# ps-auxw/CLI-P

Hardware: AMD Instinct MI355X
Metric: images/sec ViT-B/32 encode (higher is better)
Workload: dtype bf16

## Files before the change

cli-p_amd/csrc/encode.hip:

```cpp
#include "vit_kernels.hpp"

namespace clipmi {
namespace {

struct Ws {
    unsigned short* patches;
    float* x;
    unsigned short* h;
    unsigned short* big;
    unsigned short* pooled;
    int* rowidx;
    unsigned char* a8;
    float* a_scale;
    unsigned char* a_bs;
    unsigned char* x8;
    unsigned char* x8_bs;
    void* x3;
    float* ln_part;
    float* ln_leaf;
    void* x3c;
    float* partc;
    float* leafc;
    float* xc;
};
// ... 41 lines not shown
    if (t->abi_version != CLIPMI_ABI_VERSION)
        return set_err(CLIPMI_EINVAL, "%s: tower ABI %d != %d", who, t->abi_version, CLIPMI_ABI_VERSION);
    if (t->kind != kind) return set_err(CLIPMI_EINVAL, "%s: tower kind %d", who, t->kind);
    if (t->width % 128 != 0 || t->heads * 64 != t->width || t->mlp != 4 * t->width || t->embed % 128 != 0 ||
        t->width > 1024 || t->layers < 1)
        return set_err(CLIPMI_EUNSUPPORTED,
                       "%s: width=%d heads=%d mlp=%d embed=%d (need width %% 128 == 0 <= 1024, head dim 64, embed %% 128 == 0)",
                       who, t->width, t->heads, t->mlp, t->embed);
    if (t->weight_format != 0 && t->weight_format != 1)
        return set_err(CLIPMI_EINVAL, "%s: weight_format %d", who, t->weight_format);
    if (t->weight_format == 1 && t->width % 256 != 0)
        return set_err(CLIPMI_EUNSUPPORTED, "%s: fp8 weights need width %% 256 == 0 (width %d)", who, t->width);
    if (t->ln_fold != 0 && (t->ln_fold != 1 || t->width % 256 != 0))
        return set_err(CLIPMI_EINVAL, "%s: ln_fold %d needs width %% 256 == 0 (width %d)", who, t->ln_fold, t->width);
#ifndef CLIPMI_DEV
    if (t->ln_fold != 0 && t->weight_format != 0)
        return set_err(CLIPMI_EUNSUPPORTED, "%s: folded LayerNorms on FP8 weights exist in the development library only", who);
#endif
    if (t->tokens > 80 && kind == 1)
        return set_err(CLIPMI_EUNSUPPORTED, "%s: %d tokens (causal attention covers <= 80)", who, t->tokens);
    return 0;
}

template <typename T>
const T* at(const void* blob, uint64_t off) {
    return reinterpret_cast<const T*>(static_cast<const char*>(blob) + off);
}

bool encode_tail() {
    static const int mode = (int)dev_knob("CLIPMI_ENCODE_TAIL", 1);
    return mode != 0;
}

int launch_gather_rows(const void* src, void* dst, int B, int L, size_t row_bytes, hipStream_t st) {
    if (row_bytes % 16 != 0) return set_err(CLIPMI_EINVAL, "gather_rows: %zu bytes per row", row_bytes);
    const int row16 = (int)(row_bytes / 16);
    hipLaunchKernelGGL(gather_rows_kernel, dim3((unsigned)(((long long)B * row16 + 255) / 256)), dim3(256), 0, st,
                       static_cast<const uint4*>(src), static_cast<uint4*>(dst), B, L, row16);
    CLIPMI_CHECK_LAUNCH("gather_rows_kernel");
    return 0;
}

struct LayerW {
    const unsigned short *qkv_w, *out_w, *fc_w, *proj_w;
    const float *qkv_b, *out_b, *fc_b, *proj_b, *qkv_colsum, *fc_colsum, *qkv_s, *out_s, *fc_s, *proj_s, *ln1_w, *ln1_b, *ln2_w, *ln2_b;
    LayerW(const clipmi_tower* t, const void* blob, int l) {
        const uint64_t lb = t->off_layers + (uint64_t)l * t->layer_stride;
        auto f = [&](uint64_t lo) { return at<float>(blob, lb + lo); };
        auto h = [&](uint64_t lo) { return at<unsigned short>(blob, lb + lo); };
        qkv_w = h(t->lo_qkv_w); out_w = h(t->lo_out_w); fc_w = h(t->lo_fc_w); proj_w = h(t->lo_proj_w);
        qkv_b = f(t->ln_fold ? t->lo_qkv_cb : t->lo_qkv_b); fc_b = f(t->ln_fold ? t->lo_fc_cb : t->lo_fc_b);
        out_b = f(t->lo_out_b); proj_b = f(t->lo_proj_b); qkv_colsum = f(t->lo_qkv_colsum); fc_colsum = f(t->lo_fc_colsum);
        qkv_s = f(t->lo_qkv_s); out_s = f(t->lo_out_s); fc_s = f(t->lo_fc_s); proj_s = f(t->lo_proj_s);
        ln1_w = f(t->lo_ln1_w); ln1_b = f(t->lo_ln1_b); ln2_w = f(t->lo_ln2_w); ln2_b = f(t->lo_ln2_b);
    }
};

GemmArgs linear(const void* A, size_t lda_bytes, const unsigned short* W, const float* bias, int M, int N, int K, void* out) {
    GemmArgs g{};
    g.A = static_cast<const unsigned short*>(A); g.lda_bytes = (unsigned)lda_bytes; g.W = W; g.bias = bias;
    g.M = M; g.N = N; g.K = K; g.out = out;
    return g;
}

struct Resid { const float* x; const void* x3; long long row_step; };

// ... 1 lines not shown
    const clipmi_tower* t; const void* blob; const Ws& w; int B, causal; hipStream_t st; GemmProbe* probe; bool tail; int W, L, M, last;
};

int tail_plain(const Blocks& c, const LayerW& lw, Resid& r) {
    const Ws& w = c.w; const int B = c.B, W = c.W;
    if (int rc = launch_gather_rows(w.x, w.xc, B, c.L, (size_t)W * 4, c.st)) return rc;
    if (int rc = launch_gemm_algo(linear(w.h, (size_t)c.L * W * 2, lw.out_w, lw.out_b, B, W, W, w.xc), EPI_BIAS_RESID_F32, 0, c.st, nullptr)) return rc;
    LnArgs ln2{w.xc, lw.ln2_w, lw.ln2_b, w.h, nullptr, 1, B, W, 1};
    if (int rc = launch_layernorm(ln2, c.st)) return rc;
    if (int rc = launch_gemm_algo(linear(w.h, 0, lw.fc_w, lw.fc_b, B, 4 * W, W, w.big), EPI_BIAS_QGELU_BF16, 0, c.st, nullptr)) return rc;
    r = Resid{w.xc, nullptr, 1};
    return launch_gemm_algo(linear(w.big, 0, lw.proj_w, lw.proj_b, B, W, 4 * W, w.xc), EPI_BIAS_RESID_F32, 0, c.st, nullptr);
}

int blocks_plain(const Blocks& c, Resid& r) {
    const Ws& w = c.w; const int W = c.W, M = c.M;
    for (int l = 0; l <= c.last; ++l) {
        const LayerW lw(c.t, c.blob, l);
        LnArgs ln{w.x, lw.ln1_w, lw.ln1_b, w.h, nullptr, 1, M, W, 1};
        if (int rc = launch_layernorm(ln, c.st)) return rc;
        if (int rc = launch_gemm_algo(linear(w.h, 0, lw.qkv_w, lw.qkv_b, M, 3 * W, W, w.big), EPI_BIAS_BF16, 0, c.st, c.probe)) return rc;
        if (int rc = launch_attention(w.big, w.h, c.B, c.L, c.t->heads, c.causal, ATTN_DEFAULT, c.st)) return rc;
        if (c.tail && l == c.last) return tail_plain(c, lw, r);
        if (int rc = launch_gemm_algo(linear(w.h, 0, lw.out_w, lw.out_b, M, W, W, w.x), EPI_BIAS_RESID_F32, 0, c.st, c.probe)) return rc;
        ln.w = lw.ln2_w; ln.b = lw.ln2_b;
        if (int rc = launch_layernorm(ln, c.st)) return rc;
        if (int rc = launch_gemm_algo(linear(w.h, 0, lw.fc_w, lw.fc_b, M, 4 * W, W, w.big), EPI_BIAS_QGELU_BF16, 0, c.st, c.probe)) return rc;
        if (int rc = launch_gemm_algo(linear(w.big, 0, lw.proj_w, lw.proj_b, M, W, 4 * W, w.x), EPI_BIAS_RESID_F32, 0, c.st, c.probe)) return rc;
    }
    return 0;
}

int tail_ln(const Blocks& c, const LayerW& lw, Resid& r) {
    const Ws& w = c.w; const int B = c.B, W = c.W;
    float* const leaf = w.leafc && gemm_resid_writes_leaves(B, W, W) && gemm_resid_writes_leaves(B, W, 4 * W) ? w.leafc : nullptr;
    if (int rc = launch_attention(w.big, w.h, B, c.L, c.t->heads, c.causal, ATTN_DEFAULT, c.st)) return rc;
    if (int rc = launch_gather_rows(w.x3, w.x3c, B, c.L, resid_row_bytes(W), c.st)) return rc;
    GemmArgs out = linear(w.h, (size_t)c.L * W * 2, lw.out_w, lw.out_b, B, W, W, nullptr);
    out.x3 = w.x3c; out.ln_part = w.partc; out.ln_leaf = leaf; out.tmp_f32 = w.x;
    if (int rc = launch_gemm_algo(out, EPI_BIAS_RESID_LN_F32, 0, c.st, nullptr)) return rc;
    GemmArgs fc = linear(w.x3c, resid_row_bytes(W), lw.fc_w, lw.fc_b, B, 4 * W, W, w.big);
    fc.colsum = lw.fc_colsum; fc.ln_part_in = w.partc; fc.ln_leaf_in = leaf;
    if (int rc = launch_gemm_algo(fc, EPI_LN_BIAS_QGELU_BF16, 0, c.st, nullptr)) return rc;
    GemmArgs proj = linear(w.big, 0, lw.proj_w, lw.proj_b, B, W, 4 * W, nullptr);
    proj.x3 = w.x3c; proj.ln_part = w.partc; proj.ln_leaf = leaf; proj.tmp_f32 = w.x;
    r = Resid{nullptr, w.x3c, 1};
    return launch_gemm_algo(proj, EPI_BIAS_RESID_LN_F32, 0, c.st, nullptr);
}

int blocks_ln(const Blocks& c, Resid& r) {
    const Ws& w = c.w; const int W = c.W, M = c.M;
    float* const leaf = w.ln_leaf && gemm_resid_writes_leaves(M, W, W) && gemm_resid_writes_leaves(M, W, 4 * W) ? w.ln_leaf : nullptr;
    const float* leaf_in = nullptr;
    for (int l = 0; l <= c.last; ++l) {
        const LayerW lw(c.t, c.blob, l);
        GemmArgs qkv = linear(w.x3, resid_row_bytes(W), lw.qkv_w, lw.qkv_b, M, 3 * W, W, w.big);
        qkv.colsum = lw.qkv_colsum; qkv.ln_part_in = w.ln_part; qkv.ln_leaf_in = leaf_in;
        if (int rc = launch_gemm_algo(qkv, EPI_LN_BIAS_BF16, 0, c.st, c.probe)) return rc;
        if (c.tail && l == c.last) return tail_ln(c, lw, r);
        hipEvent_t* aev = nullptr;
        if (c.probe && c.probe->mode == 2 && c.probe->n < GemmProbe::MAX) aev = &c.probe->ev[2 * c.probe->begin(GemmProbe::EPI_ATTENTION, 2, c.st, 0)];
        if (int rc = launch_attention(w.big, w.h, c.B, c.L, c.t->heads, c.causal, ATTN_DEFAULT, c.st, nullptr, nullptr, nullptr, aev)) return rc;
        GemmArgs out = linear(w.h, 0, lw.out_w, lw.out_b, M, W, W, nullptr);
        out.x3 = w.x3; out.ln_part = w.ln_part; out.ln_leaf = leaf; out.tmp_f32 = w.x;
        if (int rc = launch_gemm_algo(out, EPI_BIAS_RESID_LN_F32, 0, c.st, c.probe)) return rc;
        leaf_in = leaf;
        GemmArgs fc = linear(w.x3, resid_row_bytes(W), lw.fc_w, lw.fc_b, M, 4 * W, W, w.big);
        fc.colsum = lw.fc_colsum; fc.ln_part_in = w.ln_part; fc.ln_leaf_in = leaf_in;
        if (int rc = launch_gemm_algo(fc, EPI_LN_BIAS_QGELU_BF16, 0, c.st, c.probe)) return rc;
        GemmArgs proj = linear(w.big, 0, lw.proj_w, lw.proj_b, M, W, 4 * W, nullptr);
        proj.x3 = w.x3; proj.ln_part = w.ln_part; proj.ln_leaf = leaf; proj.tmp_f32 = w.x;
        if (int rc = launch_gemm_algo(proj, EPI_BIAS_RESID_LN_F32, 0, c.st, c.probe)) return rc;
    }
    return 0;
}

bool fp8_fuse_off() { static const bool off = dev_knob("CLIPMI_FP8_FUSE", 1) == 0; return off; }
int attention_fp8(const Blocks& c, const Ws& w) {
    bool fused = false;
    if (int rc = launch_attention(w.big, w.h, c.B, c.L, c.t->heads, c.causal, ATTN_DEFAULT, c.st, fp8_fuse_off() ? nullptr : w.a8, w.a_bs, &fused)) return rc;
// ... 46 lines not shown
        GemmArgs out = linear(w.a8, 0, lw.out_w, lw.out_b, M, W, W, w.x);
        out.a_bscale = w.a_bs; out.w_scale = lw.out_s; out.x8 = w.x8; out.x8_bs = w.x8_bs; out.ln_part = w.ln_part;
        if (int rc = launch_gemm_fp8(out, EPI_BIAS_RESID_LN8, c.st)) return rc;
        GemmArgs fc = linear(w.x8, 0, lw.fc_w, lw.fc_b, M, 4 * W, W, w.big);
        fc.a_bscale = w.x8_bs; fc.w_scale = lw.fc_s; fc.colsum = lw.fc_colsum; fc.ln_part_in = w.ln_part;
        const unsigned char* h8;
        if (int rc = fc_fp8(c, w, fc, EPI_LN_BIAS_QGELU_BF16, !fp8_fuse_off(), &h8)) return rc;
        GemmArgs proj = linear(h8, 0, lw.proj_w, lw.proj_b, M, W, 4 * W, w.x);
        proj.a_bscale = w.a_bs; proj.w_scale = lw.proj_s; proj.x8 = w.x8; proj.x8_bs = w.x8_bs; proj.ln_part = w.ln_part;
        if (int rc = launch_gemm_fp8(proj, EPI_BIAS_RESID_LN8, c.st)) return rc;
    }
    return 0;
}
#endif

int run_layers(const clipmi_tower* t, const void* blob, const Ws& w, int B, int causal, hipStream_t st, GemmProbe* probe, Resid* r) {
    const bool fp8 = t->weight_format == 1;
    const bool tail = !causal && !fp8 && (t->ln_fold ? w.x3c != nullptr : w.xc != nullptr) && encode_tail();
    const Blocks c{t, blob, w, B, causal, st, probe, tail, t->width, t->tokens, B * t->tokens, t->layers - 1};
    *r = Resid{w.x, w.x3, t->tokens};
#ifdef CLIPMI_DEV
    if (t->ln_fold && fp8) return blocks_ln_fp8(c);
#endif
    if (t->ln_fold) return blocks_ln(c, *r);
    return fp8 ? blocks_fp8(c) : blocks_plain(c, *r);
}

int run_head(const clipmi_tower* t, const void* blob, const Ws& w, const Resid& r, int B, const int* rowidx, float* out, int normalize, hipStream_t st) {
    const bool split = t->ln_fold && t->weight_format == 0;
    LnArgs ln{split ? nullptr : r.x, at<float>(blob, t->off_ln_post_w), at<float>(blob, t->off_ln_post_b), w.pooled, rowidx,
              r.row_step, B, t->width, 1};
    ln.x3 = r.x3;
    if (int rc = launch_layernorm(ln, st)) return rc;
    if (int rc = launch_gemm_algo(linear(w.pooled, 0, at<unsigned short>(blob, t->off_out_proj), nullptr, B, t->embed, t->width, out), EPI_F32, 0, st)) return rc;
    return normalize ? clipmi_l2_normalize_rows(out, B, t->embed, st) : 0;
}

}
}

using namespace clipmi;

extern "C" size_t clipmi_encode_image_workspace_bytes(const clipmi_tower* t, int B) {
    if (check_tower(t, 0, "encode_image")) return 0;
    if (B < 1) { set_err(CLIPMI_EINVAL, "encode_image: B=%d", B); return 0; }
    return carve(t, B, nullptr, ~(size_t)0, nullptr);
}

static int embed_image(const clipmi_tower* t, const void* blob_dev, const void* pixels_dev, int pix_dtype, int B, const Ws& w,
                       int algo, bool with_ln_pre, hipStream_t st) {
    const int W = t->width, L = t->tokens;
    const int grid = t->res / t->patch, np = grid * grid;
    PatchArgs pa{pixels_dev, w.patches, pix_dtype, B, t->res, t->patch, grid, np, t->patch_k};
    if (int rc = launch_patchify(pa, st)) return rc;
    GemmArgs g{};
    g.A = w.patches; g.W = at<unsigned short>(blob_dev, t->off_patch_w); g.bias = nullptr; g.out = w.x;
    g.M = B * np; g.N = W; g.K = t->patch_k; g.pos = at<float>(blob_dev, t->off_pos); g.np = np; g.L = L;
    if (int rc = launch_gemm_algo(g, EPI_PATCH_F32, algo, st)) return rc;
    hipLaunchKernelGGL(cls_rows_kernel, dim3((unsigned)(((long long)B * W + 255) / 256)), dim3(256), 0, st, w.x,
                       at<float>(blob_dev, t->off_cls), at<float>(blob_dev, t->off_pos), B, L, W);
    CLIPMI_CHECK_LAUNCH("cls_rows_kernel");
    if (!with_ln_pre) return 0;
    LnArgs ln{w.x, at<float>(blob_dev, t->off_ln_pre_w), at<float>(blob_dev, t->off_ln_pre_b), w.x, nullptr, 1, B * L, W, 0};
    const bool fold8 = t->ln_fold && t->weight_format == 1;
    if (t->ln_fold && !fold8) { ln.out_x3 = w.x3; ln.out_part = w.ln_part; }
    return launch_layernorm(ln, st);
}
// ... 208 lines not shown
```

cli-p_amd/csrc/gemm.hip:

```cpp
#include "gemm256p.hpp"
#include "gemm_skinny.hpp"
#include "gemm256f8.hpp"
#include <hip/hip_ext.h>
#include <cstdlib>
#include <type_traits>

namespace clipmi {

static_assert(plan_chip::NUM_CU == NUM_CU && plan_chip::LDS_BYTES == LDS_BYTES && plan_chip::G256_LDS == G256_LDS &&
              plan_chip::G256P_MAX_N == G256P_MAX_N, "gemm_plan.hpp restates these for host-only builds");

static const GemmKnobs& knobs() {
    static const GemmKnobs kn{(int)dev_knob("CLIPMI_GEMM_PERSIST", 1), (int)dev_knob("CLIPMI_GEMM_SPLIT", 40),
                              (int)dev_knob("CLIPMI_GEMM_SKINNY", 1), (int)dev_knob("CLIPMI_GEMM_GRID", NUM_CU)};
    return kn;
}

template <unsigned MASK, int E = 0, typename F>
static int with_epi(int epi, F&& f) {
    if constexpr (E <= EPI_BIAS_RESID_LN8) {
        if constexpr (epi_in(MASK, E))
            if (epi == E) return f(std::integral_constant<int, E>{});
        return with_epi<MASK, E + 1>(epi, f);
    }
    return set_err(CLIPMI_EINVAL, "gemm: epilogue %d is not built for this kernel", epi);
}

template <typename Kernel>
static void launch_probed(Kernel kernel, dim3 grid, dim3 block, int lds, hipStream_t st, GemmProbe* probe, int epi, int kernel_kind,
                          int K, const GemmArgs& g) {
    const int i = probe ? probe->begin(epi, kernel_kind, st, K) : 0;
    if (probe) hipExtLaunchKernelGGL(kernel, grid, block, lds, st, probe->ev[2 * i], probe->ev[2 * i + 1], 0, g);
    else hipLaunchKernelGGL(kernel, grid, block, lds, st, g);
}

static bool lds_opted(int* slots) {
    int dev = 0;
    (void)hipGetDevice(&dev);
    if (dev < 0 || dev >= 64) return false;
    if (slots[dev]) return true;
    slots[dev] = 1;
    return false;
}

template <auto KERNEL>
static int launch_g256(const GemmArgs& g, int grid, hipStream_t st, int lds_max, int lds, const char* opt_err, const char* name,
                       GemmProbe* probe = nullptr, int epi = 0, int kernel_kind = GK_256) {
// ... 4 lines not shown
    launch_probed(KERNEL, dim3(grid), dim3(512), lds, st, probe, epi, kernel_kind, g.K, g);
    CLIPMI_CHECK_LAUNCH(name);
    return 0;
}
static int grid256(const GemmArgs& g) { return (g.N / 256) * ((g.M + 255) / 256); }

template <int EPI>
static int launch_skinny(const GemmArgs& g, hipStream_t st) {
    const int nstrips = g.N / 16, mtiles = (g.M + 15) / 16;
    const int waves = nstrips * mtiles <= 4 * NUM_CU ? 1 : 4;
    const dim3 grid((nstrips + waves - 1) / waves, mtiles);
    if (g.K > 512) hipLaunchKernelGGL((gemm_skinny_kernel<EPI, 32>), grid, dim3(waves * 64), 0, st, g);
    else hipLaunchKernelGGL((gemm_skinny_kernel<EPI, 16>), grid, dim3(waves * 64), 0, st, g);
    CLIPMI_CHECK_LAUNCH("gemm_skinny_kernel");
    return 0;
}

static int launch_part(const GemmArgs& g, const GemmPart& part, hipStream_t st, GemmProbe* probe) {
    switch (part.kernel) {
        case GK_SKINNY:
            return with_epi<EPI_MASK_SKINNY>(part.epi, [&](auto e) { return launch_skinny<decltype(e)::value>(g, st); });
        case GK_128:
            return with_epi<EPI_MASK_128>(part.epi, [&](auto e) {
                constexpr int EPI = decltype(e)::value;
                launch_probed(gemm_bf16_nt_kernel<EPI>, dim3((g.N / GEMM_BN) * ((g.M + GEMM_BM - 1) / GEMM_BM)), dim3(256), GEMM_LDS_BYTES, st, probe, EPI, GK_128, g.K, g);
                CLIPMI_CHECK_LAUNCH("gemm_bf16_nt_kernel");
                return 0;
            });
        case GK_256:
            return with_epi<EPI_MASK_256>(part.epi, [&](auto e) {
                constexpr int EPI = decltype(e)::value;
                return launch_g256<gemm256_bf16_nt_kernel<EPI>>(g, grid256(g), st, G256_LDS, G256_LDS, "hipFuncSetAttribute(gemm256, %d B LDS)",
                                                                "gemm256_bf16_nt_kernel", probe, EPI);
            });
        default:
            return with_epi<EPI_MASK_256P>(part.epi, [&](auto e) {
                constexpr int EPI = decltype(e)::value;
                return launch_g256<gemm256p_bf16_nt_kernel<EPI, false>>(g, part.grid, st, LDS_BYTES, part.lds, "hipFuncSetAttribute(gemm256p, %d B LDS)",
                                                                        "gemm256p_bf16_nt_kernel", probe, EPI, GK_256P);
            });
    }
}

static GemmArgs gemm_rows(const GemmArgs& g, int epi, int row0, int rows) {
    GemmArgs b = g;
    b.M = rows;
    b.A = g.A + (size_t)row0 * gemm_lda(g);
    const size_t oe = (size_t)row0 * g.N;
    if (epi == EPI_BIAS_RESID_LN_F32) {
        b.x3 = static_cast<char*>(g.x3) + (size_t)row0 * resid_row_bytes(g.N); b.tmp_f32 = g.tmp_f32 + oe;
        b.ln_part = g.ln_part + (size_t)row0 * (g.N / 256) * 2;
    } else {
        b.out = static_cast<char*>(g.out) + oe * (epi_is_bf16_out(epi) ? 2 : 4);
    }
    if (b.ln_part_in) b.ln_part_in = g.ln_part_in + (size_t)row0 * (g.K / 256) * 2;
    return b;
}

bool gemm_resid_writes_leaves(int M, int N, int K) {
    const GemmPlan p = gemm_plan(M, N, K, EPI_BIAS_RESID_LN_F32, 0, true, false, 0, knobs());
    return !p.err && p.nparts == 1 && p.part[0].leaves;
}

int launch_gemm_algo(const GemmArgs& g, int epi, int algo, hipStream_t st, GemmProbe* probe) {
    if (epi_is_ln(epi) && ((!g.ln_part_in && !g.ln_leaf_in) || !g.colsum || !g.bias))
        return set_err(CLIPMI_EINVAL, "gemm: LN-folded epilogue %d needs ln_part_in, colsum, bias and K %% 256 == 0, K <= 1024", epi);
// ... 32 lines not shown
                                                                                      "gemm256p_bf16_nt_kernel");
            });
        case GK_F8_BSA:
            return with_epi<EPI_MASK_FP8_BSA>(epi, [&](auto e) {
                return launch_g256<gemm256f8_nt_kernel<decltype(e)::value, true, true>>(
                    g, grid256(g), st, G256_LDS + 256 * (plan_chip::FP8_BSA_MAX_K / 32), G256_LDS + 256 * (g.K / 32),
                    "hipFuncSetAttribute(gemm256f8 block-scaled)", "gemm256f8_nt_kernel(block-scaled A)");
            });
    }
    return with_epi<EPI_MASK_FP8>(epi, [&](auto e) {
        constexpr int EPI = decltype(e)::value;
        const char *opt_err = "hipFuncSetAttribute(gemm256f8, %d B LDS)", *name = "gemm256f8_nt_kernel";
        return mx ? launch_g256<gemm256f8_nt_kernel<EPI, true>>(g, grid256(g), st, G256_LDS, G256_LDS, opt_err, name)
                  : launch_g256<gemm256f8_nt_kernel<EPI, false>>(g, grid256(g), st, G256_LDS, G256_LDS, opt_err, name);
    });
}

bool gemm_fp8_emits_mx(int M, int N, int K) {
    const GemmPlan p = gemm_fp8_plan(M, N, K, EPI_BIAS_QGELU_BF16, 1, false, false, 0, knobs());
    return !p.err && p.part[0].kernel == GK_256P;
}

}

using namespace clipmi;

static GemmArgs hook_args(const void* a, const void* w, const float* bias, void* out, int M, int N, int K) {
    GemmArgs g{};
    g.A = static_cast<const unsigned short*>(a); g.W = static_cast<const unsigned short*>(w); g.bias = bias; g.out = out;
    g.M = M; g.N = N; g.K = K;
    return g;
}

extern "C" int clipmi_dbg_gemm_bf16(const void* a_dev, const void* w_dev, const float* bias_dev, void* out_dev, int M,
                                    int N, int K, int epi, void* stream) {
    const int algo = (epi >> 8) & 7;
    epi &= 0xff;
    if (epi < 0 || epi > 3) return set_err(CLIPMI_EINVAL, "dbg_gemm: epi %d", epi);
    GemmArgs g = hook_args(a_dev, w_dev, bias_dev, out_dev, M, N, K);
    static const int dbg_env = (int)dev_knob("CLIPMI_GEMM_DBG", 0);
    g.dbg = dbg_env;
    if (g.dbg & 12) { g.pos = bias_dev; g.bias = nullptr; }
    return launch_gemm_algo(g, epi, algo, as_stream(stream));
}

extern "C" int clipmi_dbg_gemm_ln(const void* x3_dev, const void* wg_dev, const float* cb_dev, const float* colsum_dev,
                                  const float* part_dev, void* out_dev, int M, int N, int K, int epi, void* stream) {
    const int algo = (epi >> 8) & 3;
    epi &= 0xff;
    if (!epi_is_ln(epi)) return set_err(CLIPMI_EINVAL, "dbg_gemm_ln: epi %d", epi);
    GemmArgs g = hook_args(x3_dev, wg_dev, cb_dev, out_dev, M, N, K);
    g.lda_bytes = (unsigned)resid_row_bytes(K); g.colsum = colsum_dev; g.ln_part_in = part_dev;
    return launch_gemm_algo(g, epi, algo, as_stream(stream));
}

extern "C" int clipmi_dbg_gemm_resid_ln_leaf(const void* a_dev, const void* w_dev, const float* bias_dev, void* x3_dev, float* leaf_dev,
                                             int M, int N, int K, void* stream) {
    if (!leaf_dev || !gemm_resid_writes_leaves(M, N, K))
        return set_err(CLIPMI_EINVAL, "dbg_gemm_resid_ln_leaf: M <= %d, N %% 256 == 0, N <= 1024, K %% 32 == 0", SKINNY_MAX_M);
    GemmArgs g = hook_args(a_dev, w_dev, bias_dev, nullptr, M, N, K);
    g.x3 = x3_dev; g.ln_leaf = leaf_dev;
    g.ln_part = leaf_dev; g.tmp_f32 = leaf_dev;
    return launch_gemm_algo(g, EPI_BIAS_RESID_LN_F32, 0, as_stream(stream));
}

extern "C" int clipmi_dbg_gemm_ln_leaf(const void* x3_dev, const void* wg_dev, const float* cb_dev, const float* colsum_dev,
                                       const float* leaf_dev, void* out_dev, int M, int N, int K, int epi, void* stream) {
    if (!epi_is_ln(epi)) return set_err(CLIPMI_EINVAL, "dbg_gemm_ln_leaf: epi %d", epi);
    GemmArgs g = hook_args(x3_dev, wg_dev, cb_dev, out_dev, M, N, K);
    g.lda_bytes = (unsigned)resid_row_bytes(K); g.colsum = colsum_dev; g.ln_leaf_in = leaf_dev;
    return launch_gemm_algo(g, epi, 0, as_stream(stream));
}

extern "C" int clipmi_dbg_gemm_resid_ln(const void* a_dev, const void* w_dev, const float* bias_dev, void* x3_dev,
                                        float* part_dev, float* tmp_dev, int M, int N, int K, int algo, void* stream) {
    GemmArgs g = hook_args(a_dev, w_dev, bias_dev, nullptr, M, N, K);
    g.x3 = x3_dev; g.ln_part = part_dev; g.tmp_f32 = tmp_dev;
    static const int dbg_env = (int)dev_knob("CLIPMI_GEMM_DBG", 0);
    g.dbg = dbg_env;
    return launch_gemm_algo(g, EPI_BIAS_RESID_LN_F32, algo & 7, as_stream(stream));
}

extern "C" int clipmi_dbg_gemm_fp8_bsa(const void* a8_dev, const void* w8_dev, const void* a_bscale_dev, const float* w_scale_dev,
                                       const float* bias_dev, void* out_dev, int M, int N, int K, int epi, void* stream) {
    GemmArgs g = hook_args(a8_dev, w8_dev, bias_dev, out_dev, M, N, K);
    g.a_bscale = static_cast<const unsigned char*>(a_bscale_dev); g.w_scale = w_scale_dev;
    return launch_gemm_fp8(g, epi, as_stream(stream), 1);
}

extern "C" int clipmi_dbg_gemm_fp8(const void* a8_dev, const void* w8_dev, const float* a_scale_dev, const float* w_scale_dev,
                                   const float* bias_dev, void* out_dev, int M, int N, int K, int epi, void* stream) {
    const int mx = (epi >> 8) & 1 ? 0 : ((epi >> 9) & 1 ? 2 : 1);
    epi &= 0xff;
    if (epi < 0 || epi > 3) return set_err(CLIPMI_EINVAL, "dbg_gemm_fp8: epi %d", epi);
    GemmArgs g = hook_args(a8_dev, w8_dev, bias_dev, out_dev, M, N, K);
    g.a_scale = a_scale_dev; g.w_scale = w_scale_dev;
    return launch_gemm_fp8(g, epi, as_stream(stream), mx);
}

extern "C" int clipmi_dbg_gemm_fp8_mxout(const void* a8_dev, const void* w8_dev, const float* a_scale_dev, const float* w_scale_dev,
                                         const float* bias_dev, void* out_dev, void* out_bscale_dev, int M, int N, int K, int epi,
                                         void* stream) {
    if (epi < 0 || epi > 3) return set_err(CLIPMI_EINVAL, "dbg_gemm_fp8_mxout: epi %d", epi);
    GemmArgs g = hook_args(a8_dev, w8_dev, bias_dev, out_dev, M, N, K);
    g.a_scale = a_scale_dev; g.w_scale = w_scale_dev; g.out_bscale = static_cast<unsigned char*>(out_bscale_dev);
    return launch_gemm_fp8(g, epi, as_stream(stream), 1);
}

static int plan_out(const GemmPlan& p, bool query, int32_t* out, int n_out) {
    if (!out || n_out < 1) return set_err(CLIPMI_EINVAL, "dbg_gemm_plan: no output array");
// ... 19 lines not shown
```

cli-p_amd/csrc/gemm_plan.hpp:

```cpp
#pragma once
#include <stdarg.h>
#include <stdio.h>
#include "../../include/clipmi.h"

namespace clipmi {

enum Epilogue {
    EPI_BIAS_BF16 = 0,
    EPI_BIAS_QGELU_BF16 = 1,
    EPI_BIAS_RESID_F32 = 2,
    EPI_F32 = 3,
    EPI_PATCH_F32 = 4,
    EPI_LN_BIAS_BF16 = 5,
    EPI_LN_BIAS_QGELU_BF16 = 6,
    EPI_BIAS_RESID_LN_F32 = 7,
    EPI_BIAS_RESID_LN8 = 8
};
constexpr bool epi_is_ln(int e) { return e == EPI_LN_BIAS_BF16 || e == EPI_LN_BIAS_QGELU_BF16; }
constexpr bool epi_is_qgelu(int e) { return e == EPI_BIAS_QGELU_BF16 || e == EPI_LN_BIAS_QGELU_BF16; }
constexpr bool epi_is_bf16_out(int e) { return e == EPI_BIAS_BF16 || e == EPI_BIAS_QGELU_BF16 || epi_is_ln(e); }

constexpr unsigned EPI_MASK_128 = 0x7f, EPI_MASK_256 = 0x7f;
constexpr unsigned EPI_MASK_256P = 0xe7, EPI_MASK_SKINNY = 0xff;
constexpr unsigned EPI_MASK_FP8 = 0x0f;
constexpr unsigned EPI_MASK_FP8_256P = 0x03;
#ifdef CLIPMI_DEV
constexpr unsigned EPI_MASK_FP8_BSA = 0x16c;
#else
constexpr unsigned EPI_MASK_FP8_BSA = 0x00c;
#endif
constexpr bool epi_in(unsigned mask, int e) { return e >= 0 && e < 32 && ((mask >> e) & 1u) != 0; }

namespace plan_chip {
constexpr int NUM_CU = 256, LDS_BYTES = 160 * 1024, G256_LDS = 128 * 1024, G256P_MAX_N = 8192, FP8_BSA_MAX_K = 4096;
}
constexpr int SKINNY_MAX_M = 128;

constexpr int g256p_lds(int epi, bool fp8, int N, int K, int dbg) {
    const int nseg = K >> 8;
    return plan_chip::G256_LDS + N * 4 * (fp8 ? 2 : 1) +
           (fp8 ? 1024 : epi_is_ln(epi) ? 1024 + 256 * nseg * 8 + (nseg < 4 ? 8 : 0) : 0) + ((dbg & 12) ? 8192 + 2048 : 0);
}

struct GemmKnobs {
    int persist = 1;
    int split = 40;
    int skinny = 1;
    int grid = plan_chip::NUM_CU;
};

enum GemmKernel { GK_128 = 0, GK_256 = 1, GK_256P = 2, GK_SKINNY = 3, GK_F8 = 4, GK_F8_BSA = 5 };

struct GemmPart {
    int rows, kernel, epi;
    bool scratch;
    bool leaves;
    int grid, lds;
};
struct GemmPlan {
    int err = 0;
    int nparts = 0;
    GemmPart part[3];
    char msg[224];
    GemmPlan& refuse(int code, const char* fmt, ...) __attribute__((format(printf, 3, 4))) {
        va_list ap; va_start(ap, fmt); vsnprintf(msg, sizeof(msg), fmt, ap); va_end(ap);
        err = code; return *this;
    }
    GemmPlan& add(int rows, int kernel, int epi, bool scratch = false, bool leaves = false, int grid = 0, int lds = 0) {
        part[nparts++] = GemmPart{rows, kernel, epi, scratch, leaves, grid, lds}; return *this;
    }
};

inline long long tiles256(int M, int N) { return (long long)(N / 256) * (((long long)M + 255) / 256); }
inline int g256p_grid(long long tiles, const GemmKnobs& kn) { return (int)(tiles < kn.grid ? tiles : kn.grid); }

inline GemmPlan gemm_plan(int M, int N, int K, int epi, int algo, bool leaf, bool leaf_in, int dbg, const GemmKnobs& kn = GemmKnobs()) {
    GemmPlan p;
    if (epi_is_ln(epi) && (K % 256 != 0 || K > 1024))
        return p.refuse(CLIPMI_EINVAL, "gemm: LN-folded epilogue %d needs ln_part_in, colsum, bias and K %% 256 == 0, K <= 1024", epi);
    if (epi == EPI_BIAS_RESID_LN_F32 && (N % 256 != 0 || N > 1024))
        return p.refuse(CLIPMI_EINVAL, "gemm: EPI_BIAS_RESID_LN_F32 needs x3 (16-byte aligned), ln_part, tmp_f32 and N %% 256 == 0, N <= 1024");
    if (algo == 5)
        return p.refuse(CLIPMI_EUNSUPPORTED, "algo 5 (W-direct gemm256, DESIGN 4.4h) was removed: measured 33-40 %% slower in round 4, commit 9acf8e2 last carried it");
#ifndef CLIPMI_DEV
    if (algo == 4) return p.refuse(CLIPMI_EUNSUPPORTED, "algo %d exists in the development build only (libclipmi_dev.so)", algo);
#else
    if (algo == 4) return p.refuse(CLIPMI_EUNSUPPORTED, "algo 4 (gemm2w, DESIGN 4.4g) was removed in round 5: measured slower in round 3, its sources are in the history");
#endif
    const bool ok256 = N % 256 == 0 && K % 64 == 0 && K >= 128;
    if (algo == 2 && !ok256) return p.refuse(CLIPMI_EINVAL, "gemm256: N=%d K=%d (need N %% 256 == 0, K %% 64 == 0, K >= 128)", N, K);
    const bool ok256p = ok256 && K % 128 == 0 && N <= plan_chip::G256P_MAX_N && epi_in(EPI_MASK_256P, epi) && K <= (1 << 20) &&
                        g256p_lds(epi, false, N, K, dbg) <= plan_chip::LDS_BYTES;
    if (algo == 3 && !ok256p)
        return p.refuse(CLIPMI_EINVAL, "gemm256p: M=%d N=%d K=%d epi=%d (need N %% 256 == 0, K %% 128 == 0, a store-only epilogue "
                        "and bias/colsum rows that fit LDS)", M, N, K, epi);
    const int lds_p = ok256p ? g256p_lds(epi, false, N, K, dbg) : 0;
    bool use256 = algo == 2 || algo == 3, use256p = algo == 3;
    while (algo == 0 && ok256 && M >= 1024) {
        const long long tiles = tiles256(M, N);
        const long long rounds = (tiles + plan_chip::NUM_CU - 1) / plan_chip::NUM_CU;
        const long long pct = K >= 2048 ? 72 : 78;
        use256 = tiles * 100 >= rounds * plan_chip::NUM_CU * pct;
        use256p = use256 && ok256p && kn.persist != 0 && (tiles > plan_chip::NUM_CU || (epi == EPI_BIAS_RESID_LN_F32 && kn.persist != 2));
        if (!(ok256p && kn.persist != 0 && tiles > plan_chip::NUM_CU && epi != EPI_PATCH_F32 && (tiles % plan_chip::NUM_CU) != 0 &&
              (tiles % plan_chip::NUM_CU) * 100 < (long long)plan_chip::NUM_CU * kn.split))
            break;
        const long long main_tiles = (tiles / plan_chip::NUM_CU) * plan_chip::NUM_CU;
        const long long rows_main = main_tiles / (N / 256) * 256;
        if (rows_main < 256 || rows_main >= M || p.nparts == 2) break;
        p.add((int)rows_main, GK_256P, epi, false, false, g256p_grid(tiles256((int)rows_main, N), kn), lds_p);
        M -= (int)rows_main;
        use256 = use256p = false;
    }
    if (M < 1) return p.refuse(CLIPMI_EINVAL, "gemm: bad arguments");
    const char* leaf_in_err = "gemm: ln_leaf_in is read by the skinny LN-folded consumers only (M <= %d)";
    if (leaf_in && p.nparts) return p.refuse(CLIPMI_EINVAL, leaf_in_err, SKINNY_MAX_M);
    const bool skinny = algo == 0 && kn.skinny != 0 && M <= SKINNY_MAX_M && N % 16 == 0 && K % 32 == 0 && K >= 32;
    const bool leaves = skinny && epi == EPI_BIAS_RESID_LN_F32 && leaf;
    if (!(skinny && (epi != EPI_BIAS_RESID_LN_F32 || leaves)) && leaf_in)
        return p.refuse(CLIPMI_EINVAL, leaf_in_err, SKINNY_MAX_M);
    const bool scratch = epi == EPI_BIAS_RESID_LN_F32 && !use256p && !leaves;
// ... 41 lines not shown
```

Baseline: 110,600.

## Add small-tile rows GEMM kernel for class-token tail and head projections

Adds a new BF16 GEMM kernel with 32- or 64-row by 64-column tiles and a 2- or 4-stage LDS ring fed by global_load_lds. It is used for the last-layer class-token GEMMs (out, fc, proj) and the output projection when the batch falls between the skinny limit and 1024 rows. At these mid-sized M the existing 256-wide tiles produce few workgroups, so smaller tiles should spread the work over more CUs. The resid-LN epilogue goes through an F32 scratch path, which adds work, and the tile size and stage count are exposed as env knobs.

New measurement: 111,200 (median of 6 runs). Within noise of the previous version (+0.5%).

```diff
diff --git a/cli-p_amd/csrc/encode.hip b/cli-p_amd/csrc/encode.hip
--- a/cli-p_amd/csrc/encode.hip
+++ b/cli-p_amd/csrc/encode.hip
@@ -97,6 +97,11 @@
     return mode != 0;
 }
 
+int tail_gemm_algo(int B) {
+    static const bool on = dev_knob("CLIPMI_TAIL_GEMM", 1) != 0;
+    return on && B > SKINNY_MAX_M && B < ROWS_END_M ? ALGO_ROWS : 0;
+}
+
 int launch_gather_rows(const void* src, void* dst, int B, int L, size_t row_bytes, hipStream_t st) {
     if (row_bytes % 16 != 0) return set_err(CLIPMI_EINVAL, "gather_rows: %zu bytes per row", row_bytes);
     const int row16 = (int)(row_bytes / 16);
@@ -164,20 +169,20 @@
 }
 
 int tail_ln(const Blocks& c, const LayerW& lw, Resid& r) {
-    const Ws& w = c.w; const int B = c.B, W = c.W;
+    const Ws& w = c.w; const int B = c.B, W = c.W, algo = tail_gemm_algo(B);
     float* const leaf = w.leafc && gemm_resid_writes_leaves(B, W, W) && gemm_resid_writes_leaves(B, W, 4 * W) ? w.leafc : nullptr;
     if (int rc = launch_attention(w.big, w.h, B, c.L, c.t->heads, c.causal, ATTN_DEFAULT, c.st)) return rc;
     if (int rc = launch_gather_rows(w.x3, w.x3c, B, c.L, resid_row_bytes(W), c.st)) return rc;
     GemmArgs out = linear(w.h, (size_t)c.L * W * 2, lw.out_w, lw.out_b, B, W, W, nullptr);
     out.x3 = w.x3c; out.ln_part = w.partc; out.ln_leaf = leaf; out.tmp_f32 = w.x;
-    if (int rc = launch_gemm_algo(out, EPI_BIAS_RESID_LN_F32, 0, c.st, nullptr)) return rc;
+    if (int rc = launch_gemm_algo(out, EPI_BIAS_RESID_LN_F32, algo, c.st, nullptr)) return rc;
     GemmArgs fc = linear(w.x3c, resid_row_bytes(W), lw.fc_w, lw.fc_b, B, 4 * W, W, w.big);
     fc.colsum = lw.fc_colsum; fc.ln_part_in = w.partc; fc.ln_leaf_in = leaf;
-    if (int rc = launch_gemm_algo(fc, EPI_LN_BIAS_QGELU_BF16, 0, c.st, nullptr)) return rc;
+    if (int rc = launch_gemm_algo(fc, EPI_LN_BIAS_QGELU_BF16, algo, c.st, nullptr)) return rc;
     GemmArgs proj = linear(w.big, 0, lw.proj_w, lw.proj_b, B, W, 4 * W, nullptr);
     proj.x3 = w.x3c; proj.ln_part = w.partc; proj.ln_leaf = leaf; proj.tmp_f32 = w.x;
     r = Resid{nullptr, w.x3c, 1};
-    return launch_gemm_algo(proj, EPI_BIAS_RESID_LN_F32, 0, c.st, nullptr);
+    return launch_gemm_algo(proj, EPI_BIAS_RESID_LN_F32, algo, c.st, nullptr);
 }
 
 int blocks_ln(const Blocks& c, Resid& r) {
@@ -290,7 +295,8 @@
               r.row_step, B, t->width, 1};
     ln.x3 = r.x3;
     if (int rc = launch_layernorm(ln, st)) return rc;
-    if (int rc = launch_gemm_algo(linear(w.pooled, 0, at<unsigned short>(blob, t->off_out_proj), nullptr, B, t->embed, t->width, out), EPI_F32, 0, st)) return rc;
+    if (int rc = launch_gemm_algo(linear(w.pooled, 0, at<unsigned short>(blob, t->off_out_proj), nullptr, B, t->embed, t->width, out), EPI_F32,
+                                  t->weight_format == 0 ? tail_gemm_algo(B) : 0, st)) return rc;
     return normalize ? clipmi_l2_normalize_rows(out, B, t->embed, st) : 0;
 }
 
diff --git a/cli-p_amd/csrc/gemm.hip b/cli-p_amd/csrc/gemm.hip
--- a/cli-p_amd/csrc/gemm.hip
+++ b/cli-p_amd/csrc/gemm.hip
@@ -1,6 +1,7 @@
 #include "gemm256p.hpp"
 #include "gemm_skinny.hpp"
 #include "gemm256f8.hpp"
+#include "gemm_rows.hpp"
 #include <hip/hip_ext.h>
 #include <cstdlib>
 #include <type_traits>
@@ -9,10 +10,12 @@
 
 static_assert(plan_chip::NUM_CU == NUM_CU && plan_chip::LDS_BYTES == LDS_BYTES && plan_chip::G256_LDS == G256_LDS &&
               plan_chip::G256P_MAX_N == G256P_MAX_N, "gemm_plan.hpp restates these for host-only builds");
+static_assert(ROWS_BN == GROWS_BN && rows_lds(32, 2) == grows_lds_bytes(32, 2) && rows_lds(64, 4) == grows_lds_bytes(64, 4), "and the small-tile kernel's");
 
 static const GemmKnobs& knobs() {
     static const GemmKnobs kn{(int)dev_knob("CLIPMI_GEMM_PERSIST", 1), (int)dev_knob("CLIPMI_GEMM_SPLIT", 40),
-                              (int)dev_knob("CLIPMI_GEMM_SKINNY", 1), (int)dev_knob("CLIPMI_GEMM_GRID", NUM_CU)};
+                              (int)dev_knob("CLIPMI_GEMM_SKINNY", 1), (int)dev_knob("CLIPMI_GEMM_GRID", NUM_CU),
+                              (int)dev_knob("CLIPMI_GEMM_ROWS_BM", ROWS_BM), (int)dev_knob("CLIPMI_GEMM_ROWS_STAGES", ROWS_STAGES)};
     return kn;
 }
 
@@ -83,6 +86,17 @@
                 constexpr int EPI = decltype(e)::value;
                 return launch_g256<gemm256_bf16_nt_kernel<EPI>>(g, grid256(g), st, G256_LDS, G256_LDS, "hipFuncSetAttribute(gemm256, %d B LDS)",
                                                                 "gemm256_bf16_nt_kernel", probe, EPI);
+            });
+        case GK_ROWS:
+            return with_epi<EPI_MASK_ROWS>(part.epi, [&](auto e) {
+                constexpr int EPI = decltype(e)::value;
+                const dim3 grid(part.grid), block(256);
+                if (part.lds == grows_lds_bytes(32, 4)) hipLaunchKernelGGL((gemm_rows_bf16_nt_kernel<EPI, 32, 4>), grid, block, part.lds, st, g);
+                else if (part.lds == grows_lds_bytes(64, 4)) hipLaunchKernelGGL((gemm_rows_bf16_nt_kernel<EPI, 64, 4>), grid, block, part.lds, st, g);
+                else if (part.lds == grows_lds_bytes(32, 2)) hipLaunchKernelGGL((gemm_rows_bf16_nt_kernel<EPI, 32, 2>), grid, block, part.lds, st, g);
+                else hipLaunchKernelGGL((gemm_rows_bf16_nt_kernel<EPI, 64, 2>), grid, block, part.lds, st, g);
+                CLIPMI_CHECK_LAUNCH("gemm_rows_bf16_nt_kernel");
+                return 0;
             });
         default:
             return with_epi<EPI_MASK_256P>(part.epi, [&](auto e) {
@@ -181,12 +195,16 @@
     return g;
 }
 
+static unsigned hook_lda(int bits, int K) { return (unsigned)((bits >> 12) & 0xff) * 2u * (unsigned)K; }
+
 extern "C" int clipmi_dbg_gemm_bf16(const void* a_dev, const void* w_dev, const float* bias_dev, void* out_dev, int M,
                                     int N, int K, int epi, void* stream) {
     const int algo = (epi >> 8) & 7;
+    const unsigned lda = hook_lda(epi, K);
     epi &= 0xff;
     if (epi < 0 || epi > 3) return set_err(CLIPMI_EINVAL, "dbg_gemm: epi %d", epi);
     GemmArgs g = hook_args(a_dev, w_dev, bias_dev, out_dev, M, N, K);
+    g.lda_bytes = lda;
     static const int dbg_env = (int)dev_knob("CLIPMI_GEMM_DBG", 0);
     g.dbg = dbg_env;
     if (g.dbg & 12) { g.pos = bias_dev; g.bias = nullptr; }
@@ -195,7 +213,7 @@
 
 extern "C" int clipmi_dbg_gemm_ln(const void* x3_dev, const void* wg_dev, const float* cb_dev, const float* colsum_dev,
                                   const float* part_dev, void* out_dev, int M, int N, int K, int epi, void* stream) {
-    const int algo = (epi >> 8) & 3;
+    const int algo = (epi >> 8) & 7;
     epi &= 0xff;
     if (!epi_is_ln(epi)) return set_err(CLIPMI_EINVAL, "dbg_gemm_ln: epi %d", epi);
     GemmArgs g = hook_args(x3_dev, wg_dev, cb_dev, out_dev, M, N, K);
@@ -224,7 +242,7 @@
 extern "C" int clipmi_dbg_gemm_resid_ln(const void* a_dev, const void* w_dev, const float* bias_dev, void* x3_dev,
                                         float* part_dev, float* tmp_dev, int M, int N, int K, int algo, void* stream) {
     GemmArgs g = hook_args(a_dev, w_dev, bias_dev, nullptr, M, N, K);
-    g.x3 = x3_dev; g.ln_part = part_dev; g.tmp_f32 = tmp_dev;
+    g.x3 = x3_dev; g.ln_part = part_dev; g.tmp_f32 = tmp_dev; g.lda_bytes = hook_lda(algo, K);
     static const int dbg_env = (int)dev_knob("CLIPMI_GEMM_DBG", 0);
     g.dbg = dbg_env;
     return launch_gemm_algo(g, EPI_BIAS_RESID_LN_F32, algo & 7, as_stream(stream));
diff --git a/cli-p_amd/csrc/gemm_plan.hpp b/cli-p_amd/csrc/gemm_plan.hpp
--- a/cli-p_amd/csrc/gemm_plan.hpp
+++ b/cli-p_amd/csrc/gemm_plan.hpp
@@ -22,6 +22,7 @@
 
 constexpr unsigned EPI_MASK_128 = 0x7f, EPI_MASK_256 = 0x7f;
 constexpr unsigned EPI_MASK_256P = 0xe7, EPI_MASK_SKINNY = 0xff;
+constexpr unsigned EPI_MASK_ROWS = 0x48;
 constexpr unsigned EPI_MASK_FP8 = 0x0f;
 constexpr unsigned EPI_MASK_FP8_256P = 0x03;
 #ifdef CLIPMI_DEV
@@ -35,6 +36,8 @@
 constexpr int NUM_CU = 256, LDS_BYTES = 160 * 1024, G256_LDS = 128 * 1024, G256P_MAX_N = 8192, FP8_BSA_MAX_K = 4096;
 }
 constexpr int SKINNY_MAX_M = 128;
+constexpr int ALGO_ROWS = 6, ROWS_END_M = 1024, ROWS_BN = 64, ROWS_BM = 32, ROWS_STAGES = 4;
+constexpr int rows_lds(int bm, int stages) { return stages * (bm + ROWS_BN) * 64 * 2; }
 
 constexpr int g256p_lds(int epi, bool fp8, int N, int K, int dbg) {
     const int nseg = K >> 8;
@@ -47,9 +50,11 @@
     int split = 40;
     int skinny = 1;
     int grid = plan_chip::NUM_CU;
+    int rows_bm = ROWS_BM;
+    int rows_stages = ROWS_STAGES;
 };
 
-enum GemmKernel { GK_128 = 0, GK_256 = 1, GK_256P = 2, GK_SKINNY = 3, GK_F8 = 4, GK_F8_BSA = 5 };
+enum GemmKernel { GK_128 = 0, GK_256 = 1, GK_256P = 2, GK_SKINNY = 3, GK_F8 = 4, GK_F8_BSA = 5, GK_ROWS = 6 };
 
 struct GemmPart {
     int rows, kernel, epi;
@@ -87,6 +92,17 @@
 #else
     if (algo == 4) return p.refuse(CLIPMI_EUNSUPPORTED, "algo 4 (gemm2w, DESIGN 4.4g) was removed in round 5: measured slower in round 3, its sources are in the history");
 #endif
+    if (algo == ALGO_ROWS) {
+        if (N < 1 || K < 1 || N % ROWS_BN != 0 || K % 64 != 0 || M <= SKINNY_MAX_M || M >= ROWS_END_M)
+            return p.refuse(CLIPMI_EINVAL, "gemm_rows: M=%d N=%d K=%d (need %d < M < %d, N %% %d == 0, K %% 64 == 0)", M, N, K, SKINNY_MAX_M,
+                            ROWS_END_M, ROWS_BN);
+        if (leaf_in) return p.refuse(CLIPMI_EINVAL, "gemm: ln_leaf_in is read by the skinny LN-folded consumers only (M <= %d)", SKINNY_MAX_M);
+        const bool scratch = epi == EPI_BIAS_RESID_LN_F32;
+        const int ran = scratch ? (int)EPI_F32 : epi;
+        if (!epi_in(EPI_MASK_ROWS, ran)) return p.refuse(CLIPMI_EINVAL, "gemm_rows: epilogue %d", ran);
+        const int bm = kn.rows_bm == 64 ? 64 : ROWS_BM;
+        return p.add(M, GK_ROWS, ran, scratch, false, (N / ROWS_BN) * ((M + bm - 1) / bm), rows_lds(bm, kn.rows_stages == 2 ? 2 : ROWS_STAGES));
+    }
     const bool ok256 = N % 256 == 0 && K % 64 == 0 && K >= 128;
     if (algo == 2 && !ok256) return p.refuse(CLIPMI_EINVAL, "gemm256: N=%d K=%d (need N %% 256 == 0, K %% 64 == 0, K >= 128)", N, K);
     const bool ok256p = ok256 && K % 128 == 0 && N <= plan_chip::G256P_MAX_N && epi_in(EPI_MASK_256P, epi) && K <= (1 << 20) &&
diff --git a/cli-p_amd/csrc/gemm_rows.hpp b/cli-p_amd/csrc/gemm_rows.hpp
--- /dev/null
+++ b/cli-p_amd/csrc/gemm_rows.hpp
@@ -0,0 +1,133 @@
+#pragma once
+#include "gemm.hpp"
+
+namespace clipmi {
+
+constexpr int GROWS_BN = 64, GROWS_BK = 64;
+constexpr int grows_lds_bytes(int BM, int S) { return S * (BM + GROWS_BN) * GROWS_BK * 2; }
+static_assert(grows_lds_bytes(64, 4) <= 64 * 1024, "no LDS opt-in, two workgroups or more per CU");
+
+template <int EPI, int BM, int S>
+__global__ void __launch_bounds__(256) gemm_rows_bf16_nt_kernel(GemmArgs g) {
+    static_assert(BM == 32 || BM == 64, "2 x 2 waves of (BM / 2) x 32");
+    static_assert(S == 2 || S == 4, "the ring's slot is kt & (S - 1)");
+    static_assert(EPI == EPI_F32 || EPI == EPI_LN_BIAS_QGELU_BF16, "the class-token tail's epilogues");
+    constexpr int A_BYTES = BM * GROWS_BK * 2, W_BYTES = GROWS_BN * GROWS_BK * 2, BUF_BYTES = A_BYTES + W_BYTES;
+    constexpr int WM = BM / 2, MT = WM / 16, NT = 2;
+    constexpr int AP = BM / 32;
+    constexpr int AHEAD = (AP + 2) * (S - 2);
+    extern __shared__ __attribute__((aligned(16))) char smem[];
+    const int tid = threadIdx.x;
+    const int lane = tid & 63;
+    const int wave = __builtin_amdgcn_readfirstlane(tid >> 6);
+    const int wm = wave >> 1, wn = wave & 1;
+    const int fr = lane & 15, fg = lane >> 4;
+
+    const int ntn = g.N / GROWS_BN;
+    int bm, bn;
+    gemm_tile_coords(blockIdx.x, gridDim.x, (g.M + BM - 1) / BM, ntn, 8, 8, bm, bn);
+    const int m0 = bm * BM, n0 = bn * GROWS_BN;
+    const int K = g.K;
+
+    const int srow = lane >> 3, spos = lane & 7;
+    const unsigned short* a_src[AP];
+    const unsigned short* w_src[2];
+#pragma unroll
+    for (int i = 0; i < AP; ++i) {
+        const int row = (wave * AP + i) * 8 + srow;
+        int am = m0 + row;
+        am = am < g.M ? am : g.M - 1;
+        a_src[i] = g.A + (size_t)am * gemm_lda(g) + (spos ^ (row & 7)) * 8;
+    }
+#pragma unroll
+    for (int i = 0; i < 2; ++i) {
+        const int row = (wave * 2 + i) * 8 + srow;
+        w_src[i] = g.W + (size_t)(n0 + row) * K + (spos ^ (row & 7)) * 8;
+    }
+    auto stage = [&](int kt, int buf) {
+        char* abase = smem + buf * BUF_BYTES + wave * AP * 1024;
+        char* bbase = smem + buf * BUF_BYTES + A_BYTES + wave * 2 * 1024;
+#pragma unroll
+        for (int i = 0; i < AP; ++i)
+            __builtin_amdgcn_global_load_lds((const __attribute__((address_space(1))) void*)(a_src[i] + kt * GROWS_BK),
+                                             (__attribute__((address_space(3))) void*)(abase + i * 1024), 16, 0, 0);
+#pragma unroll
+        for (int i = 0; i < 2; ++i)
+            __builtin_amdgcn_global_load_lds((const __attribute__((address_space(1))) void*)(w_src[i] + kt * GROWS_BK),
+                                             (__attribute__((address_space(3))) void*)(bbase + i * 1024), 16, 0, 0);
+    };
+
+    f32x4 acc[MT][NT];
+#pragma unroll
+    for (int i = 0; i < MT; ++i)
+#pragma unroll
+        for (int j = 0; j < NT; ++j) acc[i][j] = f32x4{0.f, 0.f, 0.f, 0.f};
+
+    const int sw = fr & 7;
+    const int a_off = (wm * WM + fr) * 128;
+    const int b_off = A_BYTES + (wn * 32 + fr) * 128;
+    const int c0 = ((0 + fg) ^ sw) * 16, c1 = ((4 + fg) ^ sw) * 16;
+
+    const int nk = K / GROWS_BK;
+#pragma unroll
+    for (int s = 0; s < S - 1; ++s)
+        if (s < nk) stage(s, s);
+    for (int kt = 0; kt < nk; ++kt) {
+        if (kt + S - 2 < nk) asm volatile("s_waitcnt vmcnt(%0) lgkmcnt(0)\n\ts_barrier" ::"n"(AHEAD) : "memory");
+        else asm volatile("s_waitcnt vmcnt(0) lgkmcnt(0)\n\ts_barrier" ::: "memory");
+        if (kt + S - 1 < nk) stage(kt + S - 1, (kt + S - 1) & (S - 1));
+        const char* base = smem + (kt & (S - 1)) * BUF_BYTES;
+        bf16x8 af[MT][2], wf[NT][2];
+#pragma unroll
+        for (int t = 0; t < MT; ++t) {
+            af[t][0] = *reinterpret_cast<const bf16x8*>(base + a_off + t * 2048 + c0);
+            af[t][1] = *reinterpret_cast<const bf16x8*>(base + a_off + t * 2048 + c1);
+        }
+#pragma unroll
+        for (int t = 0; t < NT; ++t) {
+            wf[t][0] = *reinterpret_cast<const bf16x8*>(base + b_off + t * 2048 + c0);
+            wf[t][1] = *reinterpret_cast<const bf16x8*>(base + b_off + t * 2048 + c1);
+        }
+#pragma unroll
+        for (int ks = 0; ks < 2; ++ks)
+#pragma unroll
+            for (int mt = 0; mt < MT; ++mt)
+#pragma unroll
+                for (int nt = 0; nt < NT; ++nt)
+                    acc[mt][nt] = __builtin_amdgcn_mfma_f32_16x16x32_bf16(wf[nt][ks], af[mt][ks], acc[mt][nt], 0, 0, 0);
+    }
+
+    f32x4 bz[NT], cs[NT];
+#pragma unroll
+    for (int nt = 0; nt < NT; ++nt) {
+        const int n = n0 + wn * 32 + nt * 16 + 4 * fg;
+        bz[nt] = g.bias ? *reinterpret_cast<const f32x4*>(g.bias + n) : f32x4{0.f, 0.f, 0.f, 0.f};
+        if (epi_is_ln(EPI)) cs[nt] = *reinterpret_cast<const f32x4*>(g.colsum + n);
+    }
+#pragma unroll
+    for (int mt = 0; mt < MT; ++mt) {
+        const int m = m0 + wm * WM + mt * 16 + fr;
+        const bool valid = m < g.M;
+        const size_t orow = (size_t)(valid ? m : g.M - 1);
+        f32x2 st = {0.f, 0.f};
+        if (epi_is_ln(EPI)) {
+            const int nseg = K >> 8;
+            st = ln_row_stats(g.ln_part_in + orow * 2 * nseg, nseg, K);
+        }
+#pragma unroll
+        for (int nt = 0; nt < NT; ++nt) {
+            const int n = n0 + wn * 32 + nt * 16 + 4 * fg;
+            if (epi_is_ln(EPI)) {
+                const f32x4 v = quick_gelu4(ln_apply(acc[mt][nt], st.x, st.y, cs[nt], bz[nt]));
+                if (valid)
+                    *reinterpret_cast<uint2*>(static_cast<unsigned short*>(g.out) + orow * g.N + n) =
+                        make_uint2(pack_bf16x2(v.x, v.y), pack_bf16x2(v.z, v.w));
+            } else {
+                const f32x4 v = acc[mt][nt] + bz[nt];
+                if (valid) *reinterpret_cast<f32x4*>(static_cast<float*>(g.out) + orow * g.N + n) = v;
+            }
+        }
+    }
+}
+
+}
```
